# open-policy-agent/gatekeeper

Measured on AMD Instinct MI355X. Metric: AdmissionReview x constraint evals/sec, higher is better.
Workload: dtype u32; 1 GPU; configs[2]: pkg/audit sweep, 50 constraints x 1000000 mixed synthetic cluster objects (80% Pod, 10% Deployment, 5% Namespace, 5% Service/ConfigMap); constraints=50, reviews_total=1000000, reviews_rank0=1000000, rows_rank0=15859334, table_bytes_rank0=529437232, parallelism=1 GPU

## Files before the change

### gatekeeper_amd/csrc/device.hpp

```cpp
#pragma once
#include <cstdint>
#include <string>
#include <vector>

#include "flatten.hpp"
#include "lower.hpp"

namespace gk {

struct DevTable;
struct DevPlan;

struct EvalOptions {
  bool download = true;
  bool want_match = false;
  uint32_t list_capacity = 0;
  bool shard = false;
  bool detached = false;
  bool kernel_only = false;
  bool time_each = false;
  bool jit_wait = true;
};

struct EvalOut {
  uint32_t n_reviews = 0, n_constraints = 0, n_tiles = 0;
  std::vector<uint64_t> viol;
  std::vector<uint64_t> err;
  std::vector<uint64_t> match;
  std::vector<uint64_t> too_big;
  std::vector<uint32_t> counts;
  std::vector<uint32_t> list;
  uint32_t list_total = 0;
  uint32_t n_overflow = 0;
  float kernel_ms = 0;
  float fast_kernel_ms = 0;
  uint32_t n_launches = 0;
  uint32_t lds_bytes = 0;
  uint64_t list_bytes = 0;
  uint64_t kernel_hash = 0;
  const void *d_viol = nullptr, *d_err = nullptr, *d_counts = nullptr;
};

std::string dev_init(int device);
int dev_count();
struct DevPart;
DevPart* dev_part_upload(int device, HostTable& part);
void dev_part_free(DevPart* p);
DevTable* dev_table_assemble(int device, std::vector<DevPart*>& parts, const HostTable& meta);
void dev_table_free(DevTable* t);
DevTable* dev_table_view(DevTable* base);
uint64_t dev_table_bytes(const DevTable* t);
DevPlan* dev_plan_upload(int device, const HostPlan& fast, const HostPlan& big);
void dev_plan_free(DevPlan* p);
void dev_plan_no_jit(DevPlan* p);
void dev_eval(const DevPlan* p, const DevTable* t, const EvalOptions& opt, EvalOut* out);
void dev_topk(const DevTable* t, uint32_t nc, const std::vector<uint32_t>& order, const std::vector<uint32_t>& grp, uint32_t k, uint32_t cap,
              std::vector<uint32_t>* idx, std::vector<uint32_t>* n, std::vector<uint32_t>* ovf);
void dev_last_viol(const DevTable* t, uint32_t nc, std::vector<uint64_t>* viol);
struct DevComm;
bool dev_comm_unique_id(char id[128], std::string* err);
DevComm* dev_comm_init(int device, const char id[128], int rank, int world, std::string* err);
void dev_comm_free(DevComm* c);
int dev_comm_rank(const DevComm* c);
int dev_comm_world(const DevComm* c);
bool dev_comm_query(const DevComm* c, int* rank, int* world, std::string* err);
struct ShardInfo {
  uint32_t stride_tiles = 0;
  uint64_t slot_bytes = 0;
  std::vector<uint32_t> shard_reviews;
};
void dev_shard_setup(DevTable* t, DevComm* c, uint32_t nc, ShardInfo* info);
void dev_shard_exchange(DevTable* t, DevComm* c, uint32_t nc, uint64_t not_evaluated, std::vector<int64_t>* totals,
                        std::vector<uint64_t>* gathered , const void** d_gathered);
struct ShardExchangeStats { float exchange_ms = 0; uint64_t inbound_bytes = 0; bool overlap = false; };
ShardExchangeStats dev_shard_exchange_stats(const DevTable* t, const DevComm* c);
void dev_shard_enqueue(const DevPlan* p, DevTable* t, DevComm* c, const EvalOptions& opt, uint32_t nc, uint64_t not_evaluated, bool allow_graph);
bool dev_shard_collect(DevTable* t, DevComm* c, uint32_t nc, std::vector<int64_t>* totals, std::vector<uint64_t>* gathered, const void** d_gathered);
void dev_jit_quiesce();
void dev_jit_cache_stats(uint64_t* hits, uint64_t* compiles);
void dev_jit_cache_drop_memory();
const char* dev_jit_cache_dir();
void dev_jit_prefetch(const DevPlan* p, const DevTable* t);
void dev_eval_launch(const DevPlan* p, const DevTable* t, const EvalOptions& opt);
void dev_eval_finish(const DevPlan* p, const DevTable* t, const EvalOptions& opt, EvalOut* out);

}
```

### gatekeeper_amd/csrc/engine.cpp

```cpp
#include <atomic>
#include <cstring>
#include <dirent.h>
#include <algorithm>
#include <chrono>
#include <condition_variable>
#include <deque>
#include <functional>
#include <thread>
#include <map>
#include <unordered_map>
#include <unordered_set>
#include <memory>
#include <mutex>
#include <shared_mutex>
#include <sstream>

#include "../../include/gkgpu.h"
#include "codegen.hpp"
#include "device.hpp"
#include "flatten.hpp"
#include "lower.hpp"
#include "pe.hpp"
#include "regex.hpp"

// ... 1346 lines not shown
      try {
        Value v = parse_json(it.text.data(), it.text.size());
        if (!v.is_object()) { h->pub.n_unreadable++; continue; }
        nsname = obj_string(v, "metadata", "namespace");
      } catch (const std::exception&) { h->pub.n_unreadable++; continue; }
      if (!nsname.empty()) {
        auto f = ns_json.find(nsname);
        if (f == ns_json.end()) {
          Value ns = e->ns_cache.get(nsname);
          f = ns_json.emplace(nsname, ns.defined() ? to_json(ns) : std::string()).first;
        }
        if (f->second.empty()) { h->pub.n_namespace_missing++; continue; }
        it.ns_text = f->second;
      }
      kept.push_back(std::move(it));
    }
    std::vector<gk_review_in> rins(kept.size());
    for (size_t i = 0; i < kept.size(); i++) {
      gk_review_in& r = rins[i];
      memset(&r, 0, sizeof r);
      r.kind = GK_REVIEW_OBJECT;
      r.source = GK_SRC_ORIGINAL;
      r.json = kept[i].text.data(); r.json_len = kept[i].text.size();
      if (!kept[i].ns_text.empty()) {
        r.namespace_json = kept[i].ns_text.data(); r.namespace_len = kept[i].ns_text.size();
        r.ns_object_json = kept[i].ns_text.data(); r.ns_object_len = kept[i].ns_text.size();
      }
      h->names.push_back(kept[i].name);
    }
    h->statuses.assign(std::max<size_t>(1, kept.size()), GK_OK);
    int rc = gk_table_create(e, rins.data(), rins.size(), flags, h->statuses.data(), out);
    if (rc != GK_OK) return rc;
    h->statuses.resize(kept.size());
    h->pub.n_reviews = kept.size();
    h->pub.statuses = h->statuses.data();
    for (int32_t st : h->statuses) { if (st == GK_REVIEW_EXCLUDED) h->pub.n_excluded++; else if (st != GK_OK) h->pub.n_rejected++; }
    if ((*out)->texts.size() == kept.size() && !kept.empty()) (*out)->owned_text = std::make_shared<std::vector<Item>>(std::move(kept));
    for (auto& nm : h->names) h->ptrs.push_back(nm.c_str());
    h->pub.names = h->ptrs.data();
    if (info) *info = &h.release()->pub;
    return GK_OK;
  } catch (const std::exception& ex) { return fail(GK_ERR_INTERNAL, ex.what()); }
}

void gk_spool_info_free(gk_spool_info* info) { if (info) delete reinterpret_cast<SpoolHolder*>(info); }

int gk_table_get_stats(const gk_table* t, gk_table_stats* out) {
  if (!t || !out) return fail(GK_ERR_INVALID, "NULL argument");
  *out = t->stats;
  return GK_OK;
}

void gk_table_free(gk_table* t) {
  if (!t) return;
  for (DevTable* v : t->views) dev_table_free(v);
  for (DevTable* v : t->tviews) dev_table_free(v);
  dev_table_free(t->dev);
  delete t;
}

struct EvalHolder {
  gk_eval_out pub;
  uint32_t lds_bytes = 0;
  EvalOut out;
  std::vector<uint32_t> ids;
  std::vector<uint32_t> host_evaluated;
};
static void complete_on_host(gk_engine* e, gk_table* t, EvalHolder* h, bool want_match, bool want_list);

int gk_table_eval(gk_engine* e, gk_table* t, uint32_t flags, gk_eval_out** out) {
  if (!e || !t || !out) return fail(GK_ERR_INVALID, "NULL argument");
  try {
    ensure_plan(e);
    if (t->dict_gen != e->dict_reg.gen())
      return fail(GK_ERR_INVALID, "the table was flattened before a constraint with dictionary predicates was added (its <leaf>.$d rows are missing): create it again");
    if (t->pruned && t->reads_gen != e->dict_reg.reads_gen())
      return fail(GK_ERR_INVALID, "the pruned table was flattened before a constraint that reads other key paths was added (GK_TABLE_PRUNED): create it again");
    std::unique_ptr<EvalHolder> h(new EvalHolder());
    EvalOptions opt;
    opt.download = !(flags & GK_EVAL_NO_DOWNLOAD);
    opt.want_match = flags & GK_EVAL_WANT_MATCH;
    opt.time_each = (flags & GK_EVAL_TIME_EACH) != 0;
    opt.kernel_only = (flags & GK_EVAL_KERNEL_ONLY) != 0 && (flags & GK_EVAL_ASYNC) != 0;
    opt.jit_wait = t->resident || t->n_reviews >= 8192;
    {
      { std::lock_guard<std::mutex> gate(e->plan_gate); }
      std::shared_lock<std::shared_mutex> l(e->plan_rw);
      h->ids = e->plan_ids;
      if (flags & GK_EVAL_WANT_LIST) opt.list_capacity = std::max<uint32_t>(1024, t->n_reviews * 4u);
      const HostPlan* hp = nullptr;
      DevPlan* dp = nullptr;
      { std::lock_guard<std::mutex> vl(e->variants_mu); dp = plan_for_table(e, t, &hp); }
      while (t->views.size() < e->extra.size()) t->views.push_back(dev_table_view(t->dev));
      std::vector<DevPlan*> gdev(e->extra.size(), nullptr);
      { std::lock_guard<std::mutex> vl(e->variants_mu); for (size_t gi = 0; gi < e->extra.size(); gi++) { const HostPlan* gh = nullptr; gdev[gi] = plan_for_group(e, t, gi + 1, &gh); } }
      if (!(flags & GK_EVAL_COLLECT)) {
        if (!e->extra.empty() && opt.jit_wait) { dev_jit_prefetch(dp, t->dev); for (size_t gi = 0; gi < e->extra.size(); gi++) dev_jit_prefetch(gdev[gi], t->views[gi]); }
        dev_eval_launch(dp, t->dev, opt);
        for (size_t gi = 0; gi < e->extra.size(); gi++) dev_eval_launch(gdev[gi], t->views[gi], opt);
      }
      if (flags & GK_EVAL_ASYNC) {
        *out = nullptr;
        return GK_OK;
      }
      dev_eval_finish(dp, t->dev, opt, &h->out);
      h->lds_bytes = h->out.lds_bytes;
      for (size_t gi = 0; gi < e->extra.size(); gi++) {
        EvalOut og;
        dev_eval_finish(gdev[gi], t->views[gi], opt, &og);
        const uint32_t row_base = h->out.n_constraints;
        EvalOut& o = h->out;
        o.viol.insert(o.viol.end(), og.viol.begin(), og.viol.end());
        o.err.insert(o.err.end(), og.err.begin(), og.err.end());
        o.match.insert(o.match.end(), og.match.begin(), og.match.end());
        o.counts.insert(o.counts.end(), og.counts.begin(), og.counts.end());
        for (size_t k = 0; k + 1 < og.list.size(); k += 2) { o.list.push_back(og.list[k] + row_base); o.list.push_back(og.list[k + 1]); }
        for (size_t k = 0; k < og.too_big.size() && k < o.too_big.size(); k++) o.too_big[k] |= og.too_big[k];
        o.list_total += og.list_total;
        o.n_overflow += og.n_overflow;
        o.kernel_ms += og.kernel_ms; o.fast_kernel_ms += og.fast_kernel_ms;
        o.list_bytes += og.list_bytes;
        o.kernel_hash = o.kernel_hash * 1099511628211ull ^ og.kernel_hash;
        o.n_constraints += og.n_constraints;
        o.d_viol = o.d_err = o.d_counts = nullptr;
        h->ids.insert(h->ids.end(), e->extra[gi]->ids.begin(), e->extra[gi]->ids.end());
      }
    }
    if (opt.download && !(flags & GK_EVAL_DEVICE_ONLY)) complete_on_host(e, t, h.get(), opt.want_match, (flags & GK_EVAL_WANT_LIST) != 0);
    else if (opt.download) { std::lock_guard<std::mutex> hl(t->host_mu); t->host_viol.clear(); t->host_err.clear(); t->host_ids.clear(); }
    gk_eval_out& p = h->pub;
    memset(&p, 0, sizeof p);
    p.n_host_evaluated = (uint32_t)h->host_evaluated.size();
    p.host_evaluated = h->host_evaluated.empty() ? nullptr : h->host_evaluated.data();
    p.n_reviews = h->out.n_reviews; p.n_constraints = h->out.n_constraints; p.n_tiles = h->out.n_tiles;
    p.constraint_ids = h->ids.data();
    p.viol = h->out.viol.data(); p.err = h->out.err.data();
    p.match = h->out.match.empty() ? nullptr : h->out.match.data();
    p.too_big = h->out.too_big.data();
    p.counts = h->out.counts.data();
    p.list = h->out.list.data(); p.list_len = (uint32_t)(h->out.list.size() / 2); p.list_total = h->out.list_total;
    p.n_overflow = h->out.n_overflow;
    p.kernel_ms = h->out.kernel_ms; p.fast_kernel_ms = h->out.fast_kernel_ms; p.n_launches = h->out.n_launches;
    p.d_viol = h->out.d_viol; p.d_err = h->out.d_err; p.d_counts = h->out.d_counts;
    p.n_rows = t->n_rows;
    t->last_nc = p.n_constraints; t->last_ids = h->ids;
    p.lds_bytes = h->lds_bytes;
    p.kernel_text_hash = h->out.kernel_hash;
    uint64_t rows_read = 0, hdrs_read = 0, bound = 0, plan_bytes = 0;
    std::vector<uint8_t> seen(t->slot_path.size(), 0);
    uint64_t rows_once = 0, hdrs_once = 0;
    auto account = [&](const HostPlan& hp) {
      for (size_t si = 0; si < t->slot_path.size(); si++) {
        const uint32_t pth = t->slot_path[si];
        if (pth >= hp.ptab.size() || !hp.ptab[pth]) continue;
        bound++;
        uint64_t n = pth < t->path_rows.size() ? t->path_rows[pth] : 0;
        rows_read += n;
        uint32_t ent = hp.ptab[pth];
        bool str = false;
        for (uint32_t j = 0; j < (ent & 0xFF); j++) str = str || pred_needs_str(hp.path_preds[(ent >> 8) + j]);
        if (str) hdrs_read += n;
        static const bool dbg_path_rows = getenv("GK_DEBUG_PATH_ROWS") != nullptr;
        if (dbg_path_rows) fprintf(stderr, "[gkgpu paths] %-70s rows %9llu preds %3u%s\n", e->dict.to_string(pth).c_str(), (unsigned long long)n, ent & 0xFF, str ? " +hdr" : "");
        if (!(seen[si] & 1)) { seen[si] |= 1; rows_once += n; }
        if (str && !(seen[si] & 2)) { seen[si] |= 2; hdrs_once += n; }
      }
// ... 1177 lines not shown
```

### gatekeeper_amd/csrc/kernels.hip

```cpp
#include <hip/hip_runtime.h>
#include <hip/hiprtc.h>
#include <dlfcn.h>
#include <sys/stat.h>
#include <sys/wait.h>
#include <spawn.h>
#include <unistd.h>
#include <fcntl.h>
#include <array>
#include <cstring>
#include <cerrno>
#include <set>

#include <cstdio>
#include <cstdlib>
#include <atomic>
#include <condition_variable>
#include <list>
#include <map>
#include <thread>
#include <memory>
#include <mutex>
#include <stdexcept>
#include <string>
#include <vector>
// ... 838 lines not shown
    if (it != p->jit.end()) slot = it->second;
    else {
      slot = std::make_shared<JitSlot>();
      p->jit.emplace(key, slot);
      std::string src;
      try { src = assemble_jit_source(p->host_fast, rpt, rpp, kPlanHpp, kVmCoreHpp, kKernelBody, list_cap); }
      catch (const std::exception& ex) { slot->state = JitSlot::FAILED; slot->error = ex.what(); }
      if (slot->state == JitSlot::PENDING) {
        const int device = p->device;
        const uint32_t res_k = jit_res_k(p->host_fast), tot_k = jit_tot_k(p->host_fast.dims.n_constraints, (size_t)p->host_fast.dims.acc_words * rpp * 4, rpt, jit_block_of(rpt), res_k, list_cap ? list_cap : list_cap_of(jit_block_of(rpt)));
        auto build = [slot, src, device, rpt, res_k, list_cap, tot_k]() {
          std::unique_ptr<JitKernel> k;
          std::string err;
          try { k.reset(jit_build(device, src, rpt, res_k, list_cap, tot_k)); } catch (const std::exception& ex) { err = ex.what(); }
          std::lock_guard<std::mutex> l(slot->mu);
          slot->k = std::move(k);
          slot->error = err;
          slot->state = slot->k ? JitSlot::READY : JitSlot::FAILED;
          slot->cv.notify_all();
        };
        if (wait) build();
        else {
          jit_threads().reap(false);
          auto flag = std::make_shared<std::atomic<bool>>(false);
          std::thread th([build, flag]() { build(); flag->store(true); });
          std::lock_guard<std::mutex> tl(jit_threads().mu);
          jit_threads().running.emplace_back(std::move(th), flag);
        }
      }
    }
  }
  std::unique_lock<std::mutex> l(slot->mu);
  if (prefetch) return nullptr;
  if (wait) slot->cv.wait(l, [&] { return slot->state != JitSlot::PENDING; });
  if (slot->state == JitSlot::PENDING) return nullptr;
  if (slot->state == JitSlot::FAILED) {
    if (getenv("GK_JIT_STRICT")) throw std::runtime_error("plan specialisation failed: " + slot->error);
    if (!slot->error.empty()) { fprintf(stderr, "[gkgpu] plan specialisation unavailable, using the bytecode kernel: %s\n", slot->error.c_str()); slot->error.clear(); }
    return nullptr;
  }
  return slot->k.get();
}

struct Work {
  uint32_t nc = 0, n_tiles = 0, list_cap = 0;
  bool has_match = false, own_viol = true;
  uint64_t *d_viol = nullptr, *d_err = nullptr, *d_match = nullptr, *d_ovf = nullptr, *d_big = nullptr;
  uint32_t *d_counts = nullptr, *d_list = nullptr, *d_lc = nullptr, *d_done = nullptr;
  bool lc_pinned = false;
  size_t lc_pin_cap = 0;
  unsigned long long* d_prof = nullptr;
  uint32_t* d_partial = nullptr;
  uint32_t partial_cap = 0, partial_rows = 0, partial_stride = 0;
  bool partial_live = false;
  uint8_t* d_all = nullptr;
  size_t slot_bytes = 0;
  uint32_t stride_tiles = 0, shard_nc = 0;
  int shard_rank = 0, shard_world = 1;
  long long* d_totals = nullptr;
  bool overlap = false;
  uint8_t* d_all_buf[2] = {nullptr, nullptr};
  int shard_device = 0;
  hipStream_t comm_stream = nullptr;
  hipEvent_t ev_sweep[2] = {nullptr, nullptr}, ev_xchg[2] = {nullptr, nullptr};
  struct HipShardBackend;
  ShardPipe<HipShardBackend> pipe;
  void shard_teardown() {
    if (comm_stream) { stream_release(shard_device, comm_stream); comm_stream = nullptr; }
    for (int b = 0; b < 2; b++) {
      if (ev_sweep[b]) { hipEventDestroy(ev_sweep[b]); ev_sweep[b] = nullptr; }
      if (ev_xchg[b]) { hipEventDestroy(ev_xchg[b]); ev_xchg[b] = nullptr; }
    }
    pool_free(d_all_buf[0]); pool_free(d_all_buf[1]);
    d_all_buf[0] = d_all_buf[1] = nullptr; d_all = nullptr; overlap = false; pipe.overlap = false; pipe.reset();
  }
  uint32_t* last_lc = nullptr;
  unsigned long long shard_not_eval = ~0ull;
  int graph_state = 0;
  uint64_t graph_key = 0;
  hipGraphExec_t graph_exec = nullptr;
  void drop_graph() { if (graph_exec) hipGraphExecDestroy(graph_exec); graph_exec = nullptr; graph_state = 0; graph_key = 0; }
  static constexpr uint32_t LC_SLOTS = 64;
  static constexpr uint32_t LC_WORDS = 2, LC_BYTES = LC_WORDS * 4;
  hipEvent_t ev_first = nullptr, ev_last = nullptr;
  std::vector<std::pair<hipEvent_t, hipEvent_t>> evs;
  size_t pending = 0;
  bool lc_dirty = false;
  bool per_launch = false;
  uint32_t lds_bytes = 0;
  hipEvent_t ev_x0 = nullptr, ev_x1 = nullptr;
  float exchange_ms = 0;
  uint64_t kernel_hash = 0;
  uint8_t* h_pin = nullptr;
  size_t pin_cap = 0;
  uint8_t* pinned(size_t bytes) {
    if (bytes > pin_cap) {
      pinned_release(h_pin, pin_cap);
      h_pin = pinned_acquire(bytes, &pin_cap);
    }
    return h_pin;
  }
  void release() {
    drop_graph();
    pool_free(own_viol ? d_viol : nullptr); pool_free(d_err); pool_free(d_match); pool_free(d_ovf); pool_free(d_big); pool_free(d_list); if (lc_pinned) pinned_release(reinterpret_cast<uint8_t*>(d_lc), lc_pin_cap); else pool_free(d_lc); lc_pinned = false; pool_free(d_done); pool_free(d_partial);
    d_viol = d_err = d_match = d_ovf = d_big = nullptr; d_counts = d_list = d_lc = d_done = d_partial = nullptr; partial_cap = partial_rows = 0; partial_live = false; last_lc = nullptr;
  }
  ~Work() { drop_graph(); release(); pinned_release(h_pin, pin_cap); shard_teardown(); pool_free(d_totals); for (auto& e : evs) { hipEventDestroy(e.first); hipEventDestroy(e.second); } if (ev_first) hipEventDestroy(ev_first); if (ev_last) hipEventDestroy(ev_last); if (ev_x0) hipEventDestroy(ev_x0); if (ev_x1) hipEventDestroy(ev_x1); }
};

static Work* get_work(const DevTable* t, uint32_t nc, uint32_t n_tiles, const EvalOptions& opt) {
  DevTable* mt = const_cast<DevTable*>(t);
  if (!mt->work) mt->work = new Work();
  Work* w = mt->work;
  bool want_match = opt.want_match;
  if (opt.shard && (!w->d_all || w->shard_nc != nc || w->stride_tiles != n_tiles)) throw std::runtime_error("sharded evaluation without dev_shard_setup for this plan");
  if (w->nc != nc || w->n_tiles != n_tiles || w->list_cap < opt.list_capacity || (want_match && !w->has_match) || w->own_viol == opt.shard) {
    if (w->d_err) (void)hipStreamSynchronize(t->stream);
    w->release();
    const size_t bm = std::max<size_t>((size_t)nc * n_tiles, 1);
    if (opt.shard) {
      w->d_viol = reinterpret_cast<uint64_t*>(w->d_all + (size_t)w->shard_rank * w->slot_bytes);
      w->own_viol = false;
    } else {
      HIP_OK(pool_malloc(&w->d_viol, bm * 8 + std::max<size_t>(nc, 1) * 4));
      w->own_viol = true;
    }
    w->d_counts = reinterpret_cast<uint32_t*>(w->d_viol + bm);
    HIP_OK(pool_malloc(&w->d_err, bm * 8));
    if (want_match) HIP_OK(pool_malloc(&w->d_match, bm * 8));
    HIP_OK(pool_malloc(&w->d_ovf, std::max<size_t>(n_tiles, 1) * 8));
    HIP_OK(pool_malloc(&w->d_big, std::max<size_t>(n_tiles, 1) * 8));
    static const bool lc_host = !(getenv("GK_LC_PINNED") && atoi(getenv("GK_LC_PINNED")) == 0);
    if (lc_host && !opt.shard && opt.list_capacity == 0) {
      w->d_lc = reinterpret_cast<uint32_t*>(pinned_acquire((Work::LC_SLOTS + 1) * Work::LC_BYTES, &w->lc_pin_cap));
      w->lc_pinned = w->d_lc != nullptr;
    }
    if (!w->lc_pinned) HIP_OK(pool_malloc(&w->d_lc, (Work::LC_SLOTS + 1) * Work::LC_BYTES));
    HIP_OK(hipMemsetAsync(w->d_lc, 0, (Work::LC_SLOTS + 1) * Work::LC_BYTES, t->stream));
    HIP_OK(pool_malloc(&w->d_done, 4));
    HIP_OK(hipMemsetAsync(w->d_done, 0, 4, t->stream));
    if (opt.list_capacity) HIP_OK(pool_malloc(&w->d_list, (size_t)opt.list_capacity * 8));
    w->nc = nc; w->n_tiles = n_tiles; w->list_cap = opt.list_capacity; w->has_match = want_match;
  }
  return w;
}

void dev_table_free_work(DevTable* t) { delete t->work; t->work = nullptr; }

static void bind_paths(DevTable* t, DevTable::Binding* b, uint64_t plan_id, const std::vector<uint32_t>& entries) {
  if (b->plan_id == plan_id) return;
  std::vector<Bind> v;
  for (uint32_t s = 0; s < t->slot_path.size(); s++) {
    uint32_t path = t->slot_path[s];
    if (path < entries.size() && entries[path] != 0) v.push_back(Bind{s, entries[path]});
  }
  if (b->d) (void)hipStreamSynchronize(t->stream);
  pool_free(b->d);
  b->d = upload(v.data(), v.size());
  b->n = (uint32_t)v.size();
  b->plan_id = plan_id;
}

static void bind_chunks(DevTable* t, DevTable::Binding* b, uint64_t key, const std::vector<uint32_t>& entries, const std::vector<uint32_t>& cost,
                        bool generic, int block, uint32_t list_cap) {
  if (b->plan_id == key && b->lists) return;
  if (!t->h_tile_idx) throw std::runtime_error("table without a host slot index");
  std::vector<BoundPath> bound;
  for (uint32_t s = 0; s < t->slot_path.size(); s++) {
    const uint32_t path = t->slot_path[s];
    if (path >= entries.size() || entries[path] == 0) continue;
    if (generic && entries[path] > GK_DESC_ENT_MASK) throw Unsupported("plan too large for the chunk descriptors (predicate table beyond 2^17 entries)");
    bound.push_back(BoundPath{s, entries[path], path < cost.size() ? cost[path] : 1u});
  }
  const uint32_t n_groups = (t->n_reviews + t->rpt - 1) / t->rpt;
  ChunkLists cl = build_chunk_lists(t->h_tile_idx->data(), n_groups, t->n_slots, std::move(bound), list_cap, (uint32_t)(block / GK_TILE));
  if (b->lists) (void)hipStreamSynchronize(t->stream);
  pool_free(b->lists);
  b->lists = upload(cl.d.data(), cl.d.size());
  b->capg = cl.capg;
  b->list_bytes = (uint64_t)cl.d.size() * sizeof(ChunkDesc);
  b->plan_id = key;
}

static uint32_t grid_for(int device, uint32_t n_groups, size_t lds_per_group, int block) {
  static std::mutex mu;
  static std::map<int, int> cus;
  int n_cu;
  {
    std::lock_guard<std::mutex> l(mu);
    auto it = cus.find(device);
    if (it == cus.end()) {
      int v = 0;
      if (hipDeviceGetAttribute(&v, hipDeviceAttributeMultiprocessorCount, device) != hipSuccess || v <= 0) v = 256;
      it = cus.emplace(device, v).first;
    }
    n_cu = it->second;
  }
  const uint32_t all = (n_groups + 7u) / 8u * 8u;
  static const int persist = getenv("GK_PERSIST") ? atoi(getenv("GK_PERSIST")) : -1;
  if (persist == 0) return all;
  size_t per_cu = std::max<size_t>(1, std::min<size_t>(GK_LDS_PER_CU / std::max<size_t>(lds_per_group, 1), (size_t)2048 / (size_t)block));
  if (persist > 0) per_cu = (size_t)persist;
  const uint32_t fit = (uint32_t)((size_t)n_cu * per_cu + 7u) / 8u * 8u;
  return std::min(all, fit);
}

static void jit_geometry(const DevPlan* p, const DevTable* t, uint32_t* rpp_out, uint32_t* lcap_out) {
  const uint32_t rpt = t->rpt;
  uint32_t rpp = rpt;
  const size_t dyn_cap = p->want_jit ? max_dyn_lds_jit(rpt, p->res_k, 0, jit_tot_k(p->n_constraints)) : max_dyn_lds_of(rpt);
  while (rpp > (uint32_t)GK_TILE && (size_t)p->fast.dims.acc_words * rpp * 4 > dyn_cap) rpp /= 2;
  if (const char* f = getenv("GK_FORCE_RPP")) rpp = std::min<uint32_t>(rpt, std::max<uint32_t>(GK_TILE, (uint32_t)atoi(f)));
  uint32_t jit_lcap = list_cap_of(jit_block_of(rpt));
  if (p->want_jit && rpt >= 256) {
    DevTable* mt = const_cast<DevTable*>(t);
    if (mt->chunk_need_plan != p->id) { mt->chunk_need = chunk_need(p, t); mt->chunk_need_plan = p->id; }
    jit_lcap = jit_list_cap(jit_block_of(rpt), mt->chunk_need);
  }
  *rpp_out = rpp; *lcap_out = jit_lcap;
}

void dev_jit_prefetch(const DevPlan* p, const DevTable* t) {
  if (!p || !t || !p->want_jit || t->n_reviews == 0 || p->n_constraints == 0) return;
  uint32_t rpp = 0, lcap = 0;
  jit_geometry(p, t, &rpp, &lcap);
  try { (void)jit_for(const_cast<DevPlan*>(p), t->rpt, rpp, t, false, lcap, true); } catch (const std::exception&) {}
}

void dev_eval_launch(const DevPlan* p, const DevTable* t, const EvalOptions& opt) {
  const uint32_t n = t->n_reviews, nc = p->n_constraints;
  const uint32_t n_tiles = opt.shard && t->work ? t->work->stride_tiles : (n + GK_TILE - 1) / GK_TILE;
  if (n == 0 || nc == 0) return;
  Work* w = get_work(t, nc, n_tiles, opt);
  hipStream_t stream = t->stream;
  if (opt.shard && !opt.detached && w->overlap && w->comm_stream) { HIP_OK(hipStreamSynchronize(w->comm_stream)); w->pipe.pending[0] = w->pipe.pending[1] = false; }
  if (!opt.detached && w->lc_dirty && w->pending == 0) { HIP_OK(hipMemsetAsync(w->d_lc, 0, Work::LC_SLOTS * Work::LC_BYTES, stream)); w->lc_dirty = false; }
  uint32_t* lc = w->d_lc + Work::LC_WORDS * (opt.detached ? Work::LC_SLOTS : w->pending % Work::LC_SLOTS);
  if (!opt.detached && w->pending >= Work::LC_SLOTS) HIP_OK(hipMemsetAsync(lc, 0, Work::LC_BYTES, stream));
  w->last_lc = lc;
  static const bool want_prof = getenv("GK_KERNEL_PROF") != nullptr;
  if (want_prof && !w->d_prof) { HIP_OK(pool_malloc(&w->d_prof, ((size_t)n / GK_RPT_MIN + 8) * 64)); HIP_OK(hipMemsetAsync(w->d_prof, 0, ((size_t)n / GK_RPT_MIN + 8) * 64, stream)); }
  OutPtrs out{w->d_viol, w->d_err, opt.want_match ? w->d_match : nullptr, w->d_ovf, w->d_big, w->d_counts, w->d_list, lc,
              opt.list_capacity, w->d_prof, nullptr};
  const bool per_launch = !opt.detached && opt.time_each;
  if (!w->ev_first) { HIP_OK(hipEventCreate(&w->ev_first)); HIP_OK(hipEventCreate(&w->ev_last)); }
  if (per_launch && w->pending == w->evs.size()) {
    hipEvent_t a, b;
    HIP_OK(hipEventCreate(&a)); HIP_OK(hipEventCreate(&b));
    w->evs.emplace_back(a, b);
  }
  const size_t launch_no = opt.detached ? ~(size_t)0 : w->pending++;
  const uint32_t rpt = t->rpt;
  int block = gk_block_of((int)rpt);
  const uint32_t n_groups = (n + rpt - 1) / rpt;
  static const uint32_t dbg_phase = getenv("GK_DBG_PHASE") ? (uint32_t)atoi(getenv("GK_DBG_PHASE")) : 0u;
  static const uint32_t stagger = getenv("GK_STAGGER") ? (uint32_t)atoi(getenv("GK_STAGGER")) & 0xFFFu : (uint32_t)GK_STAGGER_DEFAULT;
  constexpr uint32_t stagger_mode = 0u;
  uint32_t rpp = rpt, jit_lcap = 0;
  DevTable* mt = const_cast<DevTable*>(t);
  JitKernel* jit = nullptr;
  if (mt->launch_plan == p->id && mt->launch_jit) {
    rpp = mt->launch_rpp; jit_lcap = mt->launch_lcap; jit = static_cast<JitKernel*>(mt->launch_jit);
  } else {
    jit_geometry(p, t, &rpp, &jit_lcap);
    const bool jit_wait = opt.jit_wait;
    jit = jit_for(const_cast<DevPlan*>(p), rpt, rpp, t, jit_wait, jit_lcap);
    if (jit && (size_t)p->fast.dims.acc_words * rpp * 4 > jit->max_dyn_lds) {
      while (rpp > (uint32_t)GK_TILE && (size_t)p->fast.dims.acc_words * rpp * 4 > jit->max_dyn_lds) rpp /= 2;
      jit = jit_for(const_cast<DevPlan*>(p), rpt, rpp, t, jit_wait, jit_lcap);
    }
    mt->launch_plan = p->id; mt->launch_rpp = rpp; mt->launch_lcap = jit_lcap; mt->launch_jit = jit;
  }
  if (jit) block = jit_block_of(rpt);
  else if ((size_t)p->fast.dims.acc_words * rpp * 4 > max_dyn_lds_of(rpt)) {
    while (rpp > (uint32_t)GK_TILE && (size_t)p->fast.dims.acc_words * rpp * 4 > max_dyn_lds_of(rpt)) rpp /= 2;
  }
  bind_chunks(mt, &mt->bind_fast, (p->id * 2 + (jit ? 1 : 0)) * 2048 + (uint64_t)block, jit ? p->cls : p->ptab_fast, p->path_cost, !jit, block,
              jit ? jit_lcap : list_cap_of(block));
  const size_t lds = (size_t)p->fast.dims.acc_words * rpp * 4;
  const uint32_t dbg = dbg_phase | (n_groups >= 1024u ? (stagger << 8) | (stagger_mode << 20) : 0u);
  uint32_t grid = grid_for(t->device, n_groups, lds + static_lds_of(rpt, block, jit ? p->res_k : 0, jit ? jit_lcap : 0, jit ? jit->tot_k : 0), block);
  if (opt.shard && opt.detached && w->overlap && grid < (n_groups + 7u) / 8u * 8u) {
    static const uint32_t reserve = getenv("GK_SHARD_RESERVE_WGS") ? (uint32_t)atoi(getenv("GK_SHARD_RESERVE_WGS")) / 8u * 8u : 32u;
    if (grid > reserve + 64u) grid -= reserve;
  }
  const bool fused_totals = jit && jit->tot_k >= nc && !opt.shard;
  if (jit && jit->tot_k) {
    if ((size_t)w->partial_cap < (size_t)grid * jit->tot_k) {
      if (w->d_partial) { HIP_OK(hipStreamSynchronize(stream)); pool_free(w->d_partial); w->d_partial = nullptr; }
      w->partial_cap = ((grid + 255u) / 256u * 256u) * jit->tot_k;
      HIP_OK(pool_malloc(&w->d_partial, (size_t)w->partial_cap * 4));
    }
    out.partial = w->d_partial;
    if (!opt.detached) { w->partial_rows = grid; w->partial_stride = jit->tot_k; }
  }
  if (!opt.detached) w->partial_live = fused_totals;
  w->lds_bytes = (uint32_t)lds;
  w->kernel_hash = jit ? jit->source_hash : 0;
  if (per_launch) HIP_OK(hipEventRecord(w->evs[launch_no].first, stream));
  else if (launch_no == 0) HIP_OK(hipEventRecord(w->ev_first, stream));
  if (!opt.detached) w->per_launch = per_launch;
  if (jit) {
    PlanView pv = p->fast.view();
    const Row* rows = t->rows; const StrHdr* shdr = t->shdr; const uint32_t* rflags = t->rflags;
    const uint8_t* heap = t->heap;
    const ChunkDesc* lists = t->bind_fast.lists;
    uint32_t nn = n, nt = n_tiles, dd = dbg, cg = t->bind_fast.capg, rp = rpp;
    const ConstraintSlot* slots = p->slots;
    void* args[] = {&pv, &rows, &shdr, &lists, &cg, &rflags, &heap, &nn, &nt, &slots, &out, &dd, &rp};
    HIP_OK(hipModuleLaunchKernel(jit->tiles, grid, 1, 1, block, 1, 1, (unsigned)lds, stream, args, nullptr));
  } else {
    auto fn = rpt == 64 ? gk_eval_tiles_64 : rpt == 128 ? gk_eval_tiles_128 : rpt == 256 ? gk_eval_tiles_256 : gk_eval_tiles_512;
    hipLaunchKernelGGL(fn, dim3(grid), dim3(block), lds, stream, p->fast.view(), t->rows, t->shdr, t->bind_fast.lists, t->bind_fast.capg,
                       t->rflags, t->heap, n, n_tiles, p->slots, out, dbg, rpp);
    HIP_OK(hipGetLastError());
  }
  if (per_launch) HIP_OK(hipEventRecord(w->evs[launch_no].second, stream));
  if (!opt.shard && !opt.kernel_only && !fused_totals) launch_count_rows(w->d_viol, nc, n_tiles, w->d_counts, stream, 0, true);
}

void dev_eval_finish(const DevPlan* p, const DevTable* t, const EvalOptions& opt, EvalOut* o) {
  const uint32_t n = t->n_reviews, nc = p->n_constraints;
  const uint32_t n_tiles = opt.shard && t->work ? t->work->stride_tiles : (n + GK_TILE - 1) / GK_TILE;
  o->n_reviews = n; o->n_constraints = nc; o->n_tiles = n_tiles;
  o->kernel_ms = o->fast_kernel_ms = 0;
  o->n_overflow = 0; o->list_total = 0; o->n_launches = 0;
  if (n == 0 || nc == 0) {
    o->viol.assign((size_t)nc * n_tiles, 0); o->err = o->viol; o->match = o->viol; o->too_big.assign(n_tiles, 0); o->counts.assign(nc, 0); o->list.clear();
    return;
  }
  Work* w = t->work;
  if (!w || w->pending == 0) throw std::runtime_error("dev_eval_finish without a pending launch");
  hipStream_t stream = t->stream;
  const size_t bm_words = (size_t)nc * n_tiles;
  uint32_t lc[2] = {0, 0};
  if (!w->per_launch) HIP_OK(hipEventRecord(w->ev_last, stream));
  uint32_t* d_lc_last = w->d_lc + Work::LC_WORDS * ((w->pending - 1) % Work::LC_SLOTS);
  if (w->partial_live && !opt.shard) launch_sum_partials(w->d_partial, w->partial_rows, w->partial_stride, nc, w->d_counts, stream);
  if (w->lc_pinned) {
    HIP_OK(hipStreamSynchronize(stream));
    memcpy(lc, d_lc_last, 8);
  } else if (uint8_t* pin0 = w->pinned(64)) {
    HIP_OK(hipMemcpyAsync(pin0, d_lc_last, 8, hipMemcpyDeviceToHost, stream));
    HIP_OK(hipStreamSynchronize(stream));
    memcpy(lc, pin0, 8);
  } else {
    HIP_OK(hipMemcpyAsync(lc, d_lc_last, 8, hipMemcpyDeviceToHost, stream));
    HIP_OK(hipStreamSynchronize(stream));
  }
  float total = 0;
  if (w->per_launch) { for (size_t i = 0; i < w->pending; i++) { float ms = 0; HIP_OK(hipEventElapsedTime(&ms, w->evs[i].first, w->evs[i].second)); total += ms; } }
  else HIP_OK(hipEventElapsedTime(&total, w->ev_first, w->ev_last));
  o->n_launches = (uint32_t)w->pending;
  o->lds_bytes = w->lds_bytes;
  o->kernel_hash = w->kernel_hash;
  o->list_bytes = t->bind_fast.list_bytes;
  o->fast_kernel_ms = total / (float)w->pending;
  o->kernel_ms = o->fast_kernel_ms;
  w->pending = 0;
  o->n_overflow = lc[1];
  OutPtrs out{w->d_viol, w->d_err, opt.want_match ? w->d_match : nullptr, w->d_ovf, w->d_big, w->d_counts, w->d_list, d_lc_last,
              opt.list_capacity, nullptr, nullptr};
  if (w->d_prof) {
    const size_t ng = (n + t->rpt - 1) / t->rpt;
    std::vector<unsigned long long> pr(ng * 8);
    HIP_OK(hipMemcpy(pr.data(), w->d_prof, pr.size() * 8, hipMemcpyDeviceToHost));
    if (const char* path = getenv("GK_KERNEL_PROF"); path && path[0] == '/') {
      if (FILE* f = fopen(path, "wb")) { fwrite(pr.data(), 8, pr.size(), f); fclose(f); }
    }
    double d[7] = {0}, waited = 0;
    for (size_t g = 0; g < ng; g++) { for (int k = 0; k < 6; k++) d[k] += (double)(pr[g * 8 + k + 1] - pr[g * 8 + k]); waited += (double)pr[g * 8 + 7]; }
    if (waited > 0) fprintf(stderr, "[gkgpu prof] wave 0 waited %.0f clocks per group for its rows in phase 1 (GK_PROF_WAIT)\n", waited / ng);
    fprintf(stderr, "[gkgpu prof] rpt %u groups %zu: mean clocks  zero+barrier %.0f | phase1 %.0f | barrier %.0f | bounds %.0f | formulas %.0f | outputs %.0f | group total %.0f\n",
            t->rpt, ng, d[0] / ng, d[1] / ng, d[2] / ng, d[3] / ng, d[4] / ng, d[5] / ng, (d[0] + d[1] + d[2] + d[3] + d[4] + d[5]) / ng);
  }
  if (lc[1]) {
    std::vector<uint64_t> ovf(n_tiles);
    HIP_OK(hipMemcpy(ovf.data(), w->d_ovf, (size_t)n_tiles * 8, hipMemcpyDeviceToHost));
    std::vector<uint32_t> ids;
    for (uint32_t tl = 0; tl < n_tiles; tl++) for (uint64_t m = ovf[tl]; m; m &= m - 1) ids.push_back(tl * GK_TILE + (uint32_t)__builtin_ctzll(m));
    uint32_t* d_ids = upload(ids.data(), ids.size());
    uint32_t* d_scratch;
    HIP_OK(pool_malloc(&d_scratch, ids.size() * (size_t)p->big.dims.acc_words * 4));
    hipEvent_t e1, e2;
    HIP_OK(hipEventCreate(&e1)); HIP_OK(hipEventCreate(&e2));
    HIP_OK(hipEventRecord(e1, stream));
    DevTable* mt = const_cast<DevTable*>(t);
    bind_paths(mt, &mt->bind_big, p->id, p->ptab_big);
    hipLaunchKernelGGL(gk_eval_big, dim3((uint32_t)ids.size()), dim3(GK_TILE), 0, stream, p->big.view(), t->rows, t->shdr, t->tile_idx, t->n_slots,
                       t->bind_big.d, t->bind_big.n, t->rflags, t->heap, d_ids,
                       (uint32_t)ids.size(), n_tiles, p->slots, d_scratch, out, t->rpt);
    HIP_OK(hipGetLastError());
    HIP_OK(hipEventRecord(e2, stream));
    launch_count_rows(w->d_viol, nc, n_tiles, w->d_counts, stream);
    HIP_OK(hipStreamSynchronize(stream));
    float ms = 0;
    HIP_OK(hipEventElapsedTime(&ms, e1, e2));
    o->kernel_ms += ms;
    hipEventDestroy(e1); hipEventDestroy(e2);
    pool_free(d_ids); pool_free(d_scratch);
    if (w->lc_pinned) memcpy(lc, d_lc_last, 8); else HIP_OK(hipMemcpy(lc, d_lc_last, 8, hipMemcpyDeviceToHost));
  }
  w->lc_dirty = true;
  o->list_total = lc[0];
  o->d_viol = w->d_viol; o->d_err = w->d_err; o->d_counts = w->d_counts;
  if (opt.download) {
    o->viol.resize(bm_words); o->err.resize(bm_words); o->counts.resize(nc); o->too_big.resize(n_tiles);
    if (opt.want_match) o->match.resize(bm_words);
    const uint32_t k = opt.list_capacity ? std::min(lc[0], opt.list_capacity) : 0u;
    o->list.resize((size_t)k * 2);
    struct Piece { void* dst; const void* src; size_t bytes; };
    const Piece pieces[] = {{o->viol.data(), w->d_viol, bm_words * 8}, {o->err.data(), w->d_err, bm_words * 8}, {o->counts.data(), w->d_counts, (size_t)nc * 4},
                            {o->too_big.data(), w->d_big, (size_t)n_tiles * 8}, {opt.want_match ? o->match.data() : nullptr, w->d_match, opt.want_match ? bm_words * 8 : 0},
                            {o->list.data(), w->d_list, (size_t)k * 8}};
    size_t total = 0;
    for (const Piece& pc : pieces) total += (pc.bytes + 15) & ~(size_t)15;
    uint8_t* pin = w->pinned(total);
    if (pin) {
      size_t at = 0;
      for (const Piece& pc : pieces) { if (pc.bytes) HIP_OK(hipMemcpyAsync(pin + at, pc.src, pc.bytes, hipMemcpyDeviceToHost, stream)); at += (pc.bytes + 15) & ~(size_t)15; }
      HIP_OK(hipStreamSynchronize(stream));
      at = 0;
      for (const Piece& pc : pieces) { if (pc.bytes) memcpy(pc.dst, pin + at, pc.bytes); at += (pc.bytes + 15) & ~(size_t)15; }
    } else {
      HIP_OK(hipStreamSynchronize(stream));
      for (const Piece& pc : pieces) if (pc.bytes) HIP_OK(hipMemcpy(pc.dst, pc.src, pc.bytes, hipMemcpyDeviceToHost));
    }
  } else HIP_OK(hipStreamSynchronize(stream));
}

struct Id128 { char b[128]; };
namespace {
struct Rccl {
  void* h = nullptr;
  int (*GetUniqueId)(void*) = nullptr;
  int (*CommInitRank)(void**, int, Id128, int) = nullptr;
  int (*CommDestroy)(void*) = nullptr;
  int (*AllGather)(const void*, void*, size_t, int, void*, hipStream_t) = nullptr;
  const char* (*GetErrorString)(int) = nullptr;
  int (*CommCount)(void*, int*) = nullptr;
  int (*CommUserRank)(void*, int*) = nullptr;
};
}
static Rccl* rccl_load(std::string* err) {
  static Rccl r;
  static std::mutex mu;
  std::lock_guard<std::mutex> l(mu);
  if (r.h) return &r;
  for (const char* name : {"librccl.so.1", "librccl.so", "/opt/rocm/lib/librccl.so.1"}) { r.h = dlopen(name, RTLD_NOW | RTLD_GLOBAL); if (r.h) break; }
  if (!r.h) { *err = std::string("RCCL not available: ") + dlerror(); return nullptr; }
  r.GetUniqueId = reinterpret_cast<int (*)(void*)>(dlsym(r.h, "ncclGetUniqueId"));
  r.CommInitRank = reinterpret_cast<int (*)(void**, int, Id128, int)>(dlsym(r.h, "ncclCommInitRank"));
  r.CommDestroy = reinterpret_cast<int (*)(void*)>(dlsym(r.h, "ncclCommDestroy"));
  r.AllGather = reinterpret_cast<int (*)(const void*, void*, size_t, int, void*, hipStream_t)>(dlsym(r.h, "ncclAllGather"));
  r.GetErrorString = reinterpret_cast<const char* (*)(int)>(dlsym(r.h, "ncclGetErrorString"));
  r.CommCount = reinterpret_cast<int (*)(void*, int*)>(dlsym(r.h, "ncclCommCount"));
  r.CommUserRank = reinterpret_cast<int (*)(void*, int*)>(dlsym(r.h, "ncclCommUserRank"));
  if (!r.GetUniqueId || !r.CommInitRank || !r.CommDestroy || !r.AllGather) { *err = "RCCL symbols missing"; dlclose(r.h); r.h = nullptr; return nullptr; }
  return &r;
}
constexpr int kNcclUint8 = 1;

struct DevComm { Rccl* lib = nullptr; void* comm = nullptr; int rank = 0, world = 1, device = 0; };
#define NCCL_OK(c, expr)                                                                                                   \
  do {                                                                                                                     \
    int r_ = (expr);                                                                                                       \
    if (r_ != 0) throw std::runtime_error(std::string("RCCL error: ") + ((c)->lib->GetErrorString ? (c)->lib->GetErrorString(r_) : "?") + " at " #expr); \
  } while (0)

bool dev_comm_unique_id(char id[128], std::string* err) {
  Rccl* r = rccl_load(err);
  if (!r) return false;
  if (r->GetUniqueId(id) != 0) { *err = "ncclGetUniqueId failed"; return false; }
  return true;
}
DevComm* dev_comm_init(int device, const char id[128], int rank, int world, std::string* err) {
  Rccl* r = rccl_load(err);
  if (!r) return nullptr;
  if (hipSetDevice(device) != hipSuccess) { *err = "hipSetDevice failed"; return nullptr; }
  std::unique_ptr<DevComm> c(new DevComm());
  c->lib = r; c->rank = rank; c->world = world; c->device = device;
  Id128 uid;
  memcpy(uid.b, id, 128);
  int rc = r->CommInitRank(&c->comm, world, uid, rank);
  if (rc != 0) { *err = std::string("ncclCommInitRank failed: ") + (r->GetErrorString ? r->GetErrorString(rc) : "?"); return nullptr; }
  return c.release();
}
void dev_comm_free(DevComm* c) { if (c) { if (c->comm) c->lib->CommDestroy(c->comm); delete c; } }
int dev_comm_rank(const DevComm* c) { return c->rank; }
int dev_comm_world(const DevComm* c) { return c->world; }
bool dev_comm_query(const DevComm* c, int* rank, int* world, std::string* err) {
  if (!c->lib->CommCount || !c->lib->CommUserRank) { *err = "this RCCL has no ncclCommCount / ncclCommUserRank"; return false; }
  int rc = c->lib->CommCount(c->comm, world);
  if (rc == 0) rc = c->lib->CommUserRank(c->comm, rank);
  if (rc != 0) { *err = std::string("RCCL error: ") + (c->lib->GetErrorString ? c->lib->GetErrorString(rc) : "?"); return false; }
  return true;
}

constexpr uint32_t GK_TAIL_EXTRA = 3;
__global__ void gk_slot_totals(const uint8_t* __restrict__ all, unsigned long long slot_bytes, unsigned long long tail_off, uint32_t world, uint32_t nc,
                               long long* __restrict__ totals) {
  const uint32_t i = blockIdx.x * 256u + threadIdx.x;
  if (i >= 2u * nc + GK_TAIL_EXTRA) return;
  long long s = 0;
  for (uint32_t r = 0; r < world; r++) {
    const uint8_t* tail = all + (size_t)r * slot_bytes + tail_off;
    s += i < 2u * nc ? (long long)reinterpret_cast<const uint32_t*>(tail)[i]
                     : (long long)reinterpret_cast<const unsigned long long*>(tail + (size_t)nc * 8)[i - 2u * nc];
  }
  totals[i] = s;
}
// ... 245 lines not shown
```

Measured before the change: 1313 billion evals/s.

## Cache repeat launch arguments, grow launch counters, and skip timing events when async

Adds a cached launch record so that repeated evaluations of the same plan skip get_work and the JIT lookup and call hipModuleLaunchKernel directly. Launch-counter slots now grow in extra blocks instead of wrapping, and pinned counters are zeroed on the host, which removes per-launch memsets. Timing events are recorded only when timing is wanted, and the trailing stream synchronize on the no-download path is dropped. The aim is lower host-side per-launch overhead on a throughput metric that is probably dominated by the GPU kernel. The cached path could miss changes to table state, and adding host_atomics_work alters when pinned counters are used.

```diff
diff --git a/gatekeeper_amd/csrc/device.hpp b/gatekeeper_amd/csrc/device.hpp
--- a/gatekeeper_amd/csrc/device.hpp
+++ b/gatekeeper_amd/csrc/device.hpp
@@ -19,6 +19,7 @@
   bool detached = false;
   bool kernel_only = false;
   bool time_each = false;
+  bool timed = true;
   bool jit_wait = true;
 };
 
diff --git a/gatekeeper_amd/csrc/engine.cpp b/gatekeeper_amd/csrc/engine.cpp
--- a/gatekeeper_amd/csrc/engine.cpp
+++ b/gatekeeper_amd/csrc/engine.cpp
@@ -1452,6 +1452,7 @@
     opt.want_match = flags & GK_EVAL_WANT_MATCH;
     opt.time_each = (flags & GK_EVAL_TIME_EACH) != 0;
     opt.kernel_only = (flags & GK_EVAL_KERNEL_ONLY) != 0 && (flags & GK_EVAL_ASYNC) != 0;
+    opt.timed = !(flags & GK_EVAL_ASYNC) || opt.time_each || opt.kernel_only;
     opt.jit_wait = t->resident || t->n_reviews >= 8192;
     {
       { std::lock_guard<std::mutex> gate(e->plan_gate); }
diff --git a/gatekeeper_amd/csrc/kernels.hip b/gatekeeper_amd/csrc/kernels.hip
--- a/gatekeeper_amd/csrc/kernels.hip
+++ b/gatekeeper_amd/csrc/kernels.hip
@@ -944,6 +944,37 @@
   void drop_graph() { if (graph_exec) hipGraphExecDestroy(graph_exec); graph_exec = nullptr; graph_state = 0; graph_key = 0; }
   static constexpr uint32_t LC_SLOTS = 64;
   static constexpr uint32_t LC_WORDS = 2, LC_BYTES = LC_WORDS * 4;
+  std::vector<uint32_t*> lc_more;
+  std::vector<size_t> lc_more_cap;
+  size_t lc_used = 0;
+  uint32_t* lc_slot(size_t i) const { return (i < LC_SLOTS ? d_lc : lc_more[i / LC_SLOTS - 1]) + LC_WORDS * (i % LC_SLOTS); }
+  template <class Fill> void lc_zero_used(Fill fill) {
+    if (lc_used) fill(d_lc, std::min<size_t>(lc_used, LC_SLOTS) * LC_BYTES);
+    for (size_t k = 0; k < lc_more.size() && (k + 1) * LC_SLOTS < lc_used; k++) fill(lc_more[k], std::min<size_t>(lc_used - (k + 1) * LC_SLOTS, LC_SLOTS) * LC_BYTES);
+    lc_used = 0;
+  }
+  void lc_release_more() {
+    for (size_t k = 0; k < lc_more.size(); k++) { if (lc_pinned) pinned_release(reinterpret_cast<uint8_t*>(lc_more[k]), lc_more_cap[k]); else pool_free(lc_more[k]); }
+    lc_more.clear(); lc_more_cap.clear(); lc_used = 0;
+  }
+  struct Launch {
+    uint64_t plan = 0;
+    bool want_match = false;
+    hipFunction_t fn = nullptr;
+    uint32_t grid = 0, block = 0, lds = 0, tot_k = 0;
+    uint64_t kernel_hash = 0;
+    PlanView pv{};
+    const Row* rows = nullptr; const StrHdr* shdr = nullptr; const ChunkDesc* lists = nullptr; const uint32_t* rflags = nullptr; const uint8_t* heap = nullptr;
+    const ConstraintSlot* slots = nullptr;
+    uint32_t cg = 0, nn = 0, nt = 0, dd = 0, rp = 0;
+    OutPtrs out{};
+  } cached;
+  bool timed = false;
+  size_t timed_from = 0;
+  void open_bracket(size_t launch_no, bool want, hipStream_t stream) {
+    if (launch_no == 0) timed = false;
+    if (want && !timed) { HIP_OK(hipEventRecord(ev_first, stream)); timed = true; timed_from = launch_no; }
+  }
   hipEvent_t ev_first = nullptr, ev_last = nullptr;
   std::vector<std::pair<hipEvent_t, hipEvent_t>> evs;
   size_t pending = 0;
@@ -964,11 +995,26 @@
   }
   void release() {
     drop_graph();
+    cached.plan = 0;
+    lc_release_more();
     pool_free(own_viol ? d_viol : nullptr); pool_free(d_err); pool_free(d_match); pool_free(d_ovf); pool_free(d_big); pool_free(d_list); if (lc_pinned) pinned_release(reinterpret_cast<uint8_t*>(d_lc), lc_pin_cap); else pool_free(d_lc); lc_pinned = false; pool_free(d_done); pool_free(d_partial);
     d_viol = d_err = d_match = d_ovf = d_big = nullptr; d_counts = d_list = d_lc = d_done = d_partial = nullptr; partial_cap = partial_rows = 0; partial_live = false; last_lc = nullptr;
   }
   ~Work() { drop_graph(); release(); pinned_release(h_pin, pin_cap); shard_teardown(); pool_free(d_totals); for (auto& e : evs) { hipEventDestroy(e.first); hipEventDestroy(e.second); } if (ev_first) hipEventDestroy(ev_first); if (ev_last) hipEventDestroy(ev_last); if (ev_x0) hipEventDestroy(ev_x0); if (ev_x1) hipEventDestroy(ev_x1); }
 };
+
+static bool host_atomics_work(int device) {
+  static std::mutex mu;
+  static std::map<int, bool> known;
+  std::lock_guard<std::mutex> l(mu);
+  auto it = known.find(device);
+  if (it == known.end()) {
+    int v = 0;
+    if (hipDeviceGetAttribute(&v, hipDeviceAttributeHostNativeAtomicSupported, device) != hipSuccess) { (void)hipGetLastError(); v = 0; }
+    it = known.emplace(device, v != 0).first;
+  }
+  return it->second;
+}
 
 static Work* get_work(const DevTable* t, uint32_t nc, uint32_t n_tiles, const EvalOptions& opt) {
   DevTable* mt = const_cast<DevTable*>(t);
@@ -993,7 +1039,7 @@
     HIP_OK(pool_malloc(&w->d_ovf, std::max<size_t>(n_tiles, 1) * 8));
     HIP_OK(pool_malloc(&w->d_big, std::max<size_t>(n_tiles, 1) * 8));
     static const bool lc_host = !(getenv("GK_LC_PINNED") && atoi(getenv("GK_LC_PINNED")) == 0);
-    if (lc_host && !opt.shard && opt.list_capacity == 0) {
+    if (lc_host && !opt.shard && opt.list_capacity == 0 && host_atomics_work(t->device)) {
       w->d_lc = reinterpret_cast<uint32_t*>(pinned_acquire((Work::LC_SLOTS + 1) * Work::LC_BYTES, &w->lc_pin_cap));
       w->lc_pinned = w->d_lc != nullptr;
     }
@@ -1089,16 +1135,51 @@
   try { (void)jit_for(const_cast<DevPlan*>(p), t->rpt, rpp, t, false, lcap, true); } catch (const std::exception&) {}
 }
 
+static uint32_t* lc_for_launch(Work* w, const EvalOptions& opt, hipStream_t stream) {
+  if (opt.detached) return w->d_lc + Work::LC_WORDS * Work::LC_SLOTS;
+  if (w->lc_dirty && w->pending == 0) {
+    w->lc_zero_used([&](uint32_t* at, size_t bytes) { HIP_OK(hipMemsetAsync(at, 0, bytes, stream)); });
+    w->lc_dirty = false;
+  }
+  const size_t i = w->pending;
+  while (i / Work::LC_SLOTS > w->lc_more.size()) {
+    uint32_t* blk = nullptr;
+    size_t cap = 0;
+    if (w->lc_pinned) {
+      blk = reinterpret_cast<uint32_t*>(pinned_acquire(Work::LC_SLOTS * Work::LC_BYTES, &cap));
+      if (!blk) throw std::runtime_error("no pinned memory for the launch counters");
+      memset(blk, 0, Work::LC_SLOTS * Work::LC_BYTES);
+    } else {
+      HIP_OK(pool_malloc(&blk, Work::LC_SLOTS * Work::LC_BYTES));
+      HIP_OK(hipMemsetAsync(blk, 0, Work::LC_SLOTS * Work::LC_BYTES, stream));
+    }
+    w->lc_more.push_back(blk); w->lc_more_cap.push_back(cap);
+  }
+  return w->lc_slot(i);
+}
+
 void dev_eval_launch(const DevPlan* p, const DevTable* t, const EvalOptions& opt) {
   const uint32_t n = t->n_reviews, nc = p->n_constraints;
   const uint32_t n_tiles = opt.shard && t->work ? t->work->stride_tiles : (n + GK_TILE - 1) / GK_TILE;
   if (n == 0 || nc == 0) return;
+  if (Work* cw = t->work; cw && cw->cached.plan == p->id && cw->cached.want_match == opt.want_match && !opt.shard && !opt.detached && !opt.time_each &&
+                          opt.list_capacity == 0) {
+    Work::Launch& c = cw->cached;
+    hipStream_t stream = t->stream;
+    c.out.list_count = cw->last_lc = lc_for_launch(cw, opt, stream);
+    cw->open_bracket(cw->pending++, opt.timed, stream);
+    cw->per_launch = false;
+    cw->partial_rows = c.grid; cw->partial_stride = c.tot_k; cw->partial_live = true;
+    cw->lds_bytes = c.lds; cw->kernel_hash = c.kernel_hash;
+    void* args[] = {&c.pv, &c.rows, &c.shdr, &c.lists, &c.cg, &c.rflags, &c.heap, &c.nn, &c.nt, &c.slots, &c.out, &c.dd, &c.rp};
+    HIP_OK(hipModuleLaunchKernel(c.fn, c.grid, 1, 1, c.block, 1, 1, c.lds, stream, args, nullptr));
+    return;
+  }
   Work* w = get_work(t, nc, n_tiles, opt);
+  w->cached.plan = 0;
   hipStream_t stream = t->stream;
   if (opt.shard && !opt.detached && w->overlap && w->comm_stream) { HIP_OK(hipStreamSynchronize(w->comm_stream)); w->pipe.pending[0] = w->pipe.pending[1] = false; }
-  if (!opt.detached && w->lc_dirty && w->pending == 0) { HIP_OK(hipMemsetAsync(w->d_lc, 0, Work::LC_SLOTS * Work::LC_BYTES, stream)); w->lc_dirty = false; }
-  uint32_t* lc = w->d_lc + Work::LC_WORDS * (opt.detached ? Work::LC_SLOTS : w->pending % Work::LC_SLOTS);
-  if (!opt.detached && w->pending >= Work::LC_SLOTS) HIP_OK(hipMemsetAsync(lc, 0, Work::LC_BYTES, stream));
+  uint32_t* lc = lc_for_launch(w, opt, stream);
   w->last_lc = lc;
   static const bool want_prof = getenv("GK_KERNEL_PROF") != nullptr;
   if (want_prof && !w->d_prof) { HIP_OK(pool_malloc(&w->d_prof, ((size_t)n / GK_RPT_MIN + 8) * 64)); HIP_OK(hipMemsetAsync(w->d_prof, 0, ((size_t)n / GK_RPT_MIN + 8) * 64, stream)); }
@@ -1142,15 +1223,16 @@
   const size_t lds = (size_t)p->fast.dims.acc_words * rpp * 4;
   const uint32_t dbg = dbg_phase | (n_groups >= 1024u ? (stagger << 8) | (stagger_mode << 20) : 0u);
   uint32_t grid = grid_for(t->device, n_groups, lds + static_lds_of(rpt, block, jit ? p->res_k : 0, jit ? jit_lcap : 0, jit ? jit->tot_k : 0), block);
+  const uint32_t grid_full = grid;
   if (opt.shard && opt.detached && w->overlap && grid < (n_groups + 7u) / 8u * 8u) {
     static const uint32_t reserve = getenv("GK_SHARD_RESERVE_WGS") ? (uint32_t)atoi(getenv("GK_SHARD_RESERVE_WGS")) / 8u * 8u : 32u;
     if (grid > reserve + 64u) grid -= reserve;
   }
   const bool fused_totals = jit && jit->tot_k >= nc && !opt.shard;
   if (jit && jit->tot_k) {
-    if ((size_t)w->partial_cap < (size_t)grid * jit->tot_k) {
-      if (w->d_partial) { HIP_OK(hipStreamSynchronize(stream)); pool_free(w->d_partial); w->d_partial = nullptr; }
-      w->partial_cap = ((grid + 255u) / 256u * 256u) * jit->tot_k;
+    if ((size_t)w->partial_cap < (size_t)grid_full * jit->tot_k) {
+      if (w->d_partial) { w->drop_graph(); HIP_OK(hipStreamSynchronize(stream)); pool_free(w->d_partial); w->d_partial = nullptr; }
+      w->partial_cap = ((grid_full + 255u) / 256u * 256u) * jit->tot_k;
       HIP_OK(pool_malloc(&w->d_partial, (size_t)w->partial_cap * 4));
     }
     out.partial = w->d_partial;
@@ -1159,8 +1241,8 @@
   if (!opt.detached) w->partial_live = fused_totals;
   w->lds_bytes = (uint32_t)lds;
   w->kernel_hash = jit ? jit->source_hash : 0;
-  if (per_launch) HIP_OK(hipEventRecord(w->evs[launch_no].first, stream));
-  else if (launch_no == 0) HIP_OK(hipEventRecord(w->ev_first, stream));
+  if (per_launch) { HIP_OK(hipEventRecord(w->evs[launch_no].first, stream)); if (launch_no == 0) w->timed = false; }
+  else if (!opt.detached) w->open_bracket(launch_no, opt.timed, stream);
   if (!opt.detached) w->per_launch = per_launch;
   if (jit) {
     PlanView pv = p->fast.view();
@@ -1171,6 +1253,13 @@
     const ConstraintSlot* slots = p->slots;
     void* args[] = {&pv, &rows, &shdr, &lists, &cg, &rflags, &heap, &nn, &nt, &slots, &out, &dd, &rp};
     HIP_OK(hipModuleLaunchKernel(jit->tiles, grid, 1, 1, block, 1, 1, (unsigned)lds, stream, args, nullptr));
+    if (fused_totals && !opt.detached && !per_launch && opt.list_capacity == 0 && !w->d_prof) {
+      Work::Launch& c = w->cached;
+      c.want_match = opt.want_match; c.fn = jit->tiles; c.grid = grid; c.block = (uint32_t)block; c.lds = (uint32_t)lds;
+      c.tot_k = jit->tot_k; c.kernel_hash = jit->source_hash; c.pv = pv; c.rows = rows; c.shdr = shdr; c.lists = lists; c.rflags = rflags; c.heap = heap;
+      c.slots = slots; c.cg = cg; c.nn = nn; c.nt = nt; c.dd = dd; c.rp = rp; c.out = out;
+      c.plan = p->id;
+    }
   } else {
     auto fn = rpt == 64 ? gk_eval_tiles_64 : rpt == 128 ? gk_eval_tiles_128 : rpt == 256 ? gk_eval_tiles_256 : gk_eval_tiles_512;
     hipLaunchKernelGGL(fn, dim3(grid), dim3(block), lds, stream, p->fast.view(), t->rows, t->shdr, t->bind_fast.lists, t->bind_fast.capg,
@@ -1196,8 +1285,8 @@
   hipStream_t stream = t->stream;
   const size_t bm_words = (size_t)nc * n_tiles;
   uint32_t lc[2] = {0, 0};
-  if (!w->per_launch) HIP_OK(hipEventRecord(w->ev_last, stream));
-  uint32_t* d_lc_last = w->d_lc + Work::LC_WORDS * ((w->pending - 1) % Work::LC_SLOTS);
+  if (!w->per_launch && w->timed) HIP_OK(hipEventRecord(w->ev_last, stream));
+  uint32_t* d_lc_last = w->lc_slot(w->pending - 1);
   if (w->partial_live && !opt.shard) launch_sum_partials(w->d_partial, w->partial_rows, w->partial_stride, nc, w->d_counts, stream);
   if (w->lc_pinned) {
     HIP_OK(hipStreamSynchronize(stream));
@@ -1212,12 +1301,13 @@
   }
   float total = 0;
   if (w->per_launch) { for (size_t i = 0; i < w->pending; i++) { float ms = 0; HIP_OK(hipEventElapsedTime(&ms, w->evs[i].first, w->evs[i].second)); total += ms; } }
-  else HIP_OK(hipEventElapsedTime(&total, w->ev_first, w->ev_last));
+  else if (w->timed) HIP_OK(hipEventElapsedTime(&total, w->ev_first, w->ev_last));
   o->n_launches = (uint32_t)w->pending;
+  w->lc_used = std::max(w->lc_used, w->pending);
   o->lds_bytes = w->lds_bytes;
   o->kernel_hash = w->kernel_hash;
   o->list_bytes = t->bind_fast.list_bytes;
-  o->fast_kernel_ms = total / (float)w->pending;
+  o->fast_kernel_ms = total / (float)(w->per_launch || !w->timed ? w->pending : w->pending - w->timed_from);
   o->kernel_ms = o->fast_kernel_ms;
   w->pending = 0;
   o->n_overflow = lc[1];
@@ -1263,7 +1353,9 @@
     pool_free(d_ids); pool_free(d_scratch);
     if (w->lc_pinned) memcpy(lc, d_lc_last, 8); else HIP_OK(hipMemcpy(lc, d_lc_last, 8, hipMemcpyDeviceToHost));
   }
-  w->lc_dirty = true;
+  if (w->lc_pinned) {
+    w->lc_zero_used([](uint32_t* at, size_t bytes) { memset(at, 0, bytes); });
+  } else w->lc_dirty = true;
   o->list_total = lc[0];
   o->d_viol = w->d_viol; o->d_err = w->d_err; o->d_counts = w->d_counts;
   if (opt.download) {
@@ -1288,7 +1380,7 @@
       HIP_OK(hipStreamSynchronize(stream));
       for (const Piece& pc : pieces) if (pc.bytes) HIP_OK(hipMemcpy(pc.dst, pc.src, pc.bytes, hipMemcpyDeviceToHost));
     }
-  } else HIP_OK(hipStreamSynchronize(stream));
+  }
 }
 
 struct Id128 { char b[128]; };
```

After: 1388 billion evals/s (median of 6 runs). +5.8%, better.
